# zhaodong-liu/GRAM

Hardware: AMD Instinct MI355X
Metric: users/sec @ beam=20 top-20 gen, Beauty T5-base; Recall@5 parity (higher is better)
Workload: dtype f16x3

## Files before the change

### gram_amd/csrc/gemm.hip

```cpp
#include <stdlib.h>
#include <type_traits>

#include "common.h"
#include "prof.h"

namespace {

#ifndef GRAM_PP_ABL
#define GRAM_PP_ABL 0
#endif
__device__ unsigned long long g_pp_clk[2];
constexpr int BN = 128, BK = 64;

enum { V_DMA_M64 = 31, V_DMA = 1, V_DMA_M256 = 3, V_PP = 22, V_RING_M64 = 33, V_RING_M128 = 34 };
int g_force_variant = -1;
int g_stagger = 0;
int g_pp_entry_delay = 0;
int g_pp_clk_on = 0;


__device__ __forceinline__ int swz(int row, int chunk) { return row * 128 + ((chunk ^ ((row >> 1) & 7)) << 4); }

struct EpiArgs {
  void* C;
// ... 713 lines not shown
                                       (__attribute__((address_space(3))) void*)(sw + (wave * WG + i) * 1024), 16, 0, 0);
  };

  f32x4 acc[TNW][4];
#pragma unroll
  for (int i = 0; i < TNW; ++i)
#pragma unroll
    for (int j = 0; j < 4; ++j) acc[i][j] = (f32x4){0.f, 0.f, 0.f, 0.f};

  const int nkt = K / BK;
  float rs4[4];
  if constexpr (NST >= 3) {
    constexpr int Q = AG + WG;
    static_assert(Q * (NST - 2) <= 63, "counted vmcnt");
    const char* abase = reinterpret_cast<const char*>(A + (size_t)m0 * lda);
    const char* wbase = reinterpret_cast<const char*>(W + (size_t)n0 * K);
    uint32_t a_off[AG], w_off[WG];
#pragma unroll
    for (int i = 0; i < AG; ++i) {
      const int row = (wave * AG + i) * 8 + (lane >> 3);
      a_off[i] = (uint32_t)(min(m0 + row, M - 1) - m0) * (uint32_t)lda * 2u + (uint32_t)(((lane & 7) ^ ((row >> 1) & 7)) * 16);
    }
#pragma unroll
    for (int i = 0; i < WG; ++i) {
      const int row = (wave * WG + i) * 8 + (lane >> 3);
      w_off[i] = (uint32_t)row * (uint32_t)K * 2u + (uint32_t)(((lane & 7) ^ ((row >> 1) & 7)) * 16);
    }
    const uint32_t lds0 = (uint32_t)(uintptr_t)(__attribute__((address_space(3))) char*)smem;
    const int uwave = __builtin_amdgcn_readfirstlane(wave);
    int i_slot = 0, i_kt = 0;
    auto issue = [&]() {
      const uint32_t sa = lds0 + (uint32_t)i_slot * STAGE, sw = sa + A_BYTES;
      const char* asrc = abase + (size_t)i_kt * (BK * 2);
      const char* wsrc = wbase + (size_t)i_kt * (BK * 2);
#pragma unroll
      for (int i = 0; i < AG; ++i) dma16_asm(sa + (uwave * AG + i) * 1024, a_off[i], asrc);
#pragma unroll
      for (int i = 0; i < WG; ++i) dma16_asm(sw + (uwave * WG + i) * 1024, w_off[i], wsrc);
      ++i_kt;
      i_slot = i_slot + 1 == NST ? 0 : i_slot + 1;
    };
    const int npro = min(NST - 1, nkt);
    for (int kt = 0; kt < npro; ++kt) issue();
    load_row_scales(ep, m0 + wm * 64, r16, M, rs4, n0 == 0 && wn == 0);
    int c_slot = 0;
    for (int kt = 0; kt < nkt; ++kt) {
      wait_later<Q>(min(NST - 2, nkt - 1 - kt));
      gram_sync();
      if (kt + NST - 1 < nkt) issue();
      compute_tile<TNW, X3>(smem + c_slot * STAGE, smem + c_slot * STAGE + A_BYTES, wm, wn, r16, g, acc);
      c_slot = c_slot + 1 == NST ? 0 : c_slot + 1;
    }
    gram_sync();
  } else {
  load_row_scales(ep, m0 + wm * 64, r16, M, rs4, n0 == 0 && wn == 0);
  if constexpr (NST == 1) {
    for (int kt = 0; kt < nkt; ++kt) {
      dma(kt, 0);
      gram_sync();
      compute_tile<TNW, X3>(smem, smem + A_BYTES, wm, wn, r16, g, acc);
      gram_sync();
    }
  } else {
    dma(0, 0);
    gram_sync();
    for (int kt = 0; kt < nkt; ++kt) {
      const int st = kt & 1;
      if (kt + 1 < nkt) dma(kt + 1, st ^ 1);
      compute_tile<TNW, X3>(smem + st * STAGE, smem + st * STAGE + A_BYTES, wm, wn, r16, g, acc);
      gram_sync();
    }
  }
  }
  if constexpr ((EPI == GRAM_EPI_F32_ADD || EPI == GRAM_EPI_F32) && TNW == 4 && NST != 2) {
    if (ep.nt & 4) {
      epilogue_rows64<EPI>(acc, smem + wave * 4096, m0, n0, wm, wn, lane, M, ep);
      return;
    }
  }
  epilogue<EPI, TNW>(acc, m0, n0, wm, wn, r16, g, M, ep, rs4);
}

constexpr int PP_KV_K = 100, PP_KV_V = 101;
__device__ __forceinline__ void pp_barrier() {
  asm volatile("s_barrier" ::: "memory");
  gram_chaos_point();
}

struct PPOut {
  char* c;
  char* xb;
  float* ss;
  const float* xs;
  uint32_t ldc_b;
  uint32_t ldx_b;
  uint32_t ss_nblk;
  int rows;
  int split;
  long c_ps_b;
  bool inter;
  bool nt;
  float scale;
  long q_ps;
  uint32_t q_step;
};
template <int EPI, bool FULL>
__device__ __forceinline__ void pp_store_rows_impl(f32x4 (&acc)[4][8], int j0, char* patch, const PPOut& o, int lane_, const float* rs) {
  static_assert(EPI == GRAM_EPI_BF16 || EPI == GRAM_EPI_BF16_RELU, "16-bit outputs only: the fp32 outputs go through pp_store_tile_f32");
  int lane = lane_;
  asm volatile("" : "+v"(lane));
  const int r16 = lane & 15, g = lane >> 4;
#pragma unroll
  for (int jj = 0; jj < 2; ++jj) {
    const int j = j0 + jj;
    const float sc = (rs ? rs[j * 16 + r16] : 1.f) * o.scale;
    f32x4 v[4];
#pragma unroll
    for (int i = 0; i < 4; ++i) {
      v[i] = acc[i][j] * sc;
      if constexpr (EPI == GRAM_EPI_BF16_RELU) {
#pragma unroll
        for (int e = 0; e < 4; ++e) v[i][e] = fmaxf(v[i][e], 0.f);
      }
    }
    uint2 pcs[2][4];
    if (o.split == 2) {
#pragma unroll
      for (int i = 0; i < 4; ++i) split2x4(v[i], pcs[0][i], pcs[1][i]);
    } else {
#pragma unroll
      for (int i = 0; i < 4; ++i) pcs[0][i] = pcs[1][i] = pack_bf16x4(v[i]);
    }
    for (int pc = 0; pc < o.split; ++pc) {
#pragma unroll
      for (int i = 0; i < 4; ++i) {
        const int chunk = (i * 2 + (g >> 1)) ^ (r16 & 7);
        *reinterpret_cast<uint2*>(patch + r16 * 128 + chunk * 16 + (g & 1) * 8) = pc == 0 ? pcs[0][i] : pcs[1][i];
      }
      __builtin_amdgcn_wave_barrier();
#pragma unroll
      for (int it = 0; it < 2; ++it) {
        const int row = it * 8 + (lane >> 3), c = lane & 7;
        const uint4 val = *reinterpret_cast<const uint4*>(patch + row * 128 + ((c ^ (row & 7)) * 16));
        const int mr = j * 16 + row;
        const uint32_t coff = o.inter ? (uint32_t)((c >> 2) * 128 + pc * 64 + (c & 3) * 16) : (uint32_t)(c * 16);
        if ((FULL || mr < o.rows) && (!(GRAM_PP_ABL & 16) || o.rows < -12345))
          store16(o.c + (o.inter ? 0 : pc * o.c_ps_b) + ((uint32_t)mr * o.ldc_b + coff), val, o.nt);
      }
      __builtin_amdgcn_wave_barrier();
    }
  }
}

template <int EPI>
__device__ __forceinline__ void pp_store_tile_f32(f32x4 (&acc)[4][8], char* patch, const PPOut& o, int lane_) {
  int lane = lane_;
  asm volatile("" : "+v"(lane));
  const int r16 = lane & 15, g = lane >> 4;
#pragma unroll
  for (int half = 0; half < 2; ++half) {
    f32x4 res[16];
    float xsl = 1.f;
    if constexpr (EPI == GRAM_EPI_F32_ADD) {
#pragma unroll
      for (int q = 0; q < 16; ++q) res[q] = (f32x4){0.f, 0.f, 0.f, 0.f};
      if (o.rows > 0 && o.xs) xsl = o.xs[min(half * 64 + lane, o.rows - 1)];
      if (o.rows > 0) {
#pragma unroll
        for (int q = 0; q < 16; ++q) {
          const int mr = min(half * 64 + q * 4 + (lane >> 4), o.rows - 1);
          res[q] = *reinterpret_cast<const f32x4*>(o.c + ((uint32_t)mr * o.ldc_b + (lane & 15) * 16));
        }
      }
    }
#pragma unroll
    for (int p = 0; p < 4; ++p) {
      const int j = half * 4 + p;
#pragma unroll
      for (int i = 0; i < 4; ++i) *reinterpret_cast<f32x4*>(patch + r16 * 256 + (((i * 4 + g) ^ r16) * 16)) = acc[i][j];
      __builtin_amdgcn_wave_barrier();
      float ssq4[4];
#pragma unroll
      for (int it = 0; it < 4; ++it) {
        const int row = it * 4 + (lane >> 4), c = lane & 15;
        f32x4 val = *reinterpret_cast<const f32x4*>(patch + row * 256 + ((c ^ row) * 16)) * o.scale;
        const int mr = j * 16 + row;
        float ssq = 0.f;
        const float xs_row = __shfl(xsl, p * 16 + it * 4 + (lane >> 4), 64);
        if (mr < o.rows && (!(GRAM_PP_ABL & 16) || o.rows < -12345)) {
          f32x4* pc = reinterpret_cast<f32x4*>(o.c + ((uint32_t)mr * o.ldc_b + c * 16));
          if constexpr (EPI == GRAM_EPI_F32_ADD) val += res[p * 4 + it];
          if (!(GRAM_PP_ABL & 32) || o.rows < -12345) *pc = val;
          if constexpr (EPI == GRAM_EPI_F32_ADD) {
            if (o.xb) {
              const f32x4 xv = val * xs_row;
              if (o.split == 2) {
                uint2 p0, p1;
                split2x4(xv, p0, p1);
                const bool odd = c & 1;
                const uint2 send = odd ? p0 : p1;
                uint2 recv;
                recv.x = (uint32_t)__builtin_amdgcn_mov_dpp((int)send.x, 0xB1, 0xF, 0xF, true);
                recv.y = (uint32_t)__builtin_amdgcn_mov_dpp((int)send.y, 0xB1, 0xF, 0xF, true);
                const uint4 out = odd ? make_uint4(recv.x, recv.y, p1.x, p1.y) : make_uint4(p0.x, p0.y, recv.x, recv.y);
                const uint32_t xoff = (uint32_t)((c >> 3) * 128 + (odd ? 64 : 0) + ((c & 6) * 8));
                *reinterpret_cast<uint4*>(o.xb + ((uint32_t)mr * o.ldx_b + xoff)) = out;
              } else {
                *reinterpret_cast<uint2*>(o.xb + ((uint32_t)mr * o.ldx_b + (uint32_t)(c * 8))) = pack_bf16x4(xv);
              }
              ssq = sumsq4(val);
            }
          }
        }
        ssq4[it] = ssq;
      }
      if constexpr (EPI == GRAM_EPI_F32_ADD) {
        if (o.ss) {
#pragma unroll
          for (int sh = 1; sh < 16; sh <<= 1)
#pragma unroll
            for (int it = 0; it < 4; ++it) ssq4[it] += __shfl_xor(ssq4[it], sh, 64);
          const int cc = lane & 15;
          const float mine = cc == 0 ? ssq4[0] : cc == 1 ? ssq4[1] : cc == 2 ? ssq4[2] : ssq4[3];
          const int mr = j * 16 + cc * 4 + (lane >> 4);
          if (cc < 4 && mr < o.rows) o.ss[(uint32_t)mr * o.ss_nblk] = mine;
        }
      }
      __builtin_amdgcn_wave_barrier();
    }
  }
}

template <int EPI>
__device__ __forceinline__ void pp_store_rows(f32x4 (&acc)[4][8], int j0, char* patch, const PPOut& o, int lane, const float* rs) {
  if (o.rows >= 128) pp_store_rows_impl<EPI, true>(acc, j0, patch, o, lane, rs);
  else pp_store_rows_impl<EPI, false>(acc, j0, patch, o, lane, rs);
}

template <int EPI, bool X3 = false>
__global__ __launch_bounds__(512, 1) void gemm_pp_kernel(const p16* __restrict__ A, const p16* __restrict__ W, int M, int N,
                                                         int K, int lda, EpiArgs ep, int ntiles, int stagger) {
  constexpr int TB = 256, HT = 16384;
  constexpr bool F32OUT = EPI == GRAM_EPI_F32 || EPI == GRAM_EPI_F32_ADD;
  constexpr bool KV = EPI == PP_KV_K || EPI == PP_KV_V;
  constexpr bool TRALL = EPI == PP_KV_V;
  constexpr int PATCH = 4096;
  constexpr bool LSE = EPI == GRAM_EPI_F32_LSE;
  constexpr bool TEND = F32OUT || LSE || X3;
  constexpr int RS_OFF = 8 * HT + 4 * PATCH;
  extern __shared__ __attribute__((aligned(16))) char smem[];
  const int tid = threadIdx.x;
  const int lane = tid & 63;
  const int wave = __builtin_amdgcn_readfirstlane(tid >> 6);
  const int wr = wave >> 2, wc = wave & 3;
  const int r16 = lane & 15, g = lane >> 4;
  const int ntn = KV ? N / TB / 2 : (N + TB - 1) / TB;
  auto nt_of = [&](int ntl) {
    if constexpr (KV) {
      const int it = ep.inner >> 8, blk = (int)udiv_magic((uint32_t)ntl, (uint32_t)it, ep.mg_it);
      return blk * 2 * it + (TRALL ? it : 0) + (ntl - blk * it);
    } else {
      return ntl;
    }
  };
  const int G = gridDim.x;
  const int slot = xcd_remap();
  const int xcd = blockIdx.x & 7;
  if (slot >= ntiles) return;
  const int nkt = K / BK;
  const uint32_t lds0 = (uint32_t)(uintptr_t)(__attribute__((address_space(3))) char*)smem;
  const uint32_t wave_lds = __builtin_amdgcn_readfirstlane(lds0 + wave * 2048);
  const char* const Ab = reinterpret_cast<const char*>(A);
  const char* const Wb = reinterpret_cast<const char*>(W);
  char* const patch = smem + 8 * HT + (F32OUT ? wave * PATCH : TEND ? wave * 2048 : (wave & 3) * PATCH);
  const bool has_rs = !F32OUT && ep.ss_in != nullptr;

  const int gm = (stagger >> 16) & 0xff;
  const bool clk_on = (stagger >> 30) & 1;
#ifdef GRAM_CHAOS
  const int entry_delay = (stagger >> 24) & 0x3f;
#endif
  stagger &= 0xffff;
  auto decode = [&](int tile, int& mt, int& nr) {
    if (gm <= 1) {
      mt = tile / ntn;
      nr = tile - mt * ntn;
    } else {
      const int per = gm * ntn, grp = tile / per, first = grp * gm;
      const int gs = min(gm, (M + TB - 1) / TB - first);
      const int rem = tile - grp * per;
      nr = rem / gs;
      mt = first + (rem - nr * gs);
    }
  };
  int c_tile = slot, c_kt = 0;
  const char *c_A, *c_W;
  uint32_t offA[2][2], offW[2], offW2[LSE ? 2 : 1];
  if constexpr (!LSE) {
#pragma unroll
    for (int p = 0; p < 2; ++p) {
      const int r = (wave * 2 + p) * 8 + (lane >> 3);
      const int chunk = (lane & 7) ^ ((r >> 1) & 7);
      offW[p] = ((uint32_t)((r >> 5) * 64 + (r & 31)) * (uint32_t)K + chunk * 8) * 2u;
    }
  }
  auto set_offsets = [&]() {
    int mt, nr;
    decode(c_tile, mt, nr);
    const int nt = nt_of(nr);
    c_A = Ab + (size_t)mt * TB * lda * 2;
    c_W = Wb + (size_t)nt * TB * K * 2;
    const int mleft = M - 1 - mt * TB;
    int ln = lane;
    asm volatile("" : "+v"(ln));
#pragma unroll
    for (int p = 0; p < 2; ++p) {
      const int r = (wave * 2 + p) * 8 + (ln >> 3);
      const int chunk = (ln & 7) ^ ((r >> 1) & 7);
      const int arow = (r >> 6) * 128 + (r & 63);
      offA[0][p] = ((uint32_t)min(arow, mleft) * (uint32_t)lda + chunk * 8) * 2u;
      offA[1][p] = ((uint32_t)min(arow + 64, mleft) * (uint32_t)lda + chunk * 8) * 2u;
      if constexpr (LSE) {
        const int wleft = N - 1 - nt * TB, wrow = (r >> 5) * 64 + (r & 31);
        offW[p] = ((uint32_t)min(wrow, wleft) * (uint32_t)K + chunk * 8) * 2u;
        offW2[p] = ((uint32_t)min(wrow + 32, wleft) * (uint32_t)K + chunk * 8) * 2u;
      }
    }
  };
  auto advance = [&]() {
    if (++c_kt == nkt) {
      c_kt = 0;
      if (c_tile + G < ntiles) c_tile += G;
      set_offsets();
    }
  };
  bool abl_loop = false;
  auto issue = [&](int t, int par) {
    if ((GRAM_PP_ABL & 2) && abl_loop) return;
    {
      const uint32_t dst = wave_lds + (par * 4 + t) * HT;
      if (t == 0 || t == 3) {
        const char* base = c_A + c_kt * (BK * 2);
        dma16_asm(dst, offA[t == 3][0], base);
        dma16_asm(dst + 1024, offA[t == 3][1], base);
      } else {
        if constexpr (LSE) {
          const char* base = c_W + c_kt * (BK * 2);
          dma16_asm(dst, t == 2 ? offW2[0] : offW[0], base);
          dma16_asm(dst + 1024, t == 2 ? offW2[1] : offW[1], base);
        } else {
          const char* base = c_W + c_kt * (BK * 2) + (t == 2 ? (size_t)32 * K * 2 : 0);
          dma16_asm(dst, offW[0], base);
          dma16_asm(dst + 1024, offW[1], base);
        }
      }
    }
  };

  f32x4 acc[4][8];
  p16x8 fa[2][4], fw[2][2][2];
  const char* const a_base[2] = {smem + swz(wr * 64 + r16, g), smem + swz(wr * 64 + r16, 4 + g)};
  const char* const w_base[2] = {smem + swz(wc * 32 + r16, g), smem + swz(wc * 32 + r16, 4 + g)};
  auto read_a = [&](int par, int mq) {
    if ((GRAM_PP_ABL & 4) && abl_loop) return;
    {
#pragma unroll
      for (int ks = 0; ks < 2; ++ks)
#pragma unroll
        for (int j = 0; j < 4; ++j)
          fa[ks][j] = *reinterpret_cast<const p16x8*>(a_base[ks] + (par * 4 + (mq ? 3 : 0)) * HT + j * 2048);
    }
  };
  auto read_w = [&](int par, int nq) {
    if ((GRAM_PP_ABL & 4) && abl_loop) return;
    {
#pragma unroll
      for (int ks = 0; ks < 2; ++ks)
#pragma unroll
        for (int i = 0; i < 2; ++i)
          fw[nq][ks][i] = *reinterpret_cast<const p16x8*>(w_base[ks] + (par * 4 + 1 + nq) * HT + i * 2048);
    }
  };
  constexpr int NMQ = X3 ? 24 : 16;
  auto mfma_q = [&](auto TRc, int mq, int nq, int n) {
    const int pr = n >> 3, i = (n >> 2) & 1, j = n & 3;
    const int ka = X3 ? (pr == 1 ? 1 : 0) : pr, kw = X3 ? (pr == 0 ? 1 : 0) : pr;
    f32x4& c = acc[nq * 2 + i][mq * 4 + j];
    if constexpr (decltype(TRc)::value) c = mfma16(fa[ka][j], fw[nq][kw][i], c);
    else c = mfma16(fw[nq][kw][i], fa[ka][j], c);
  };
  auto mma = [&](int mq, int nq, auto TRc) {
    __builtin_amdgcn_sched_barrier(0);
    __builtin_amdgcn_s_setprio(1);
#pragma unroll
    for (int n = 0; n < NMQ; ++n) mfma_q(TRc, mq, nq, n);
    __builtin_amdgcn_s_setprio(0);
    __builtin_amdgcn_sched_barrier(0);
    pp_barrier();
  };
  auto mma_st = [&](int mq, int nq, auto TRc, auto J0c, const PPOut& o, const float* rs, auto FULLc) {
    constexpr bool FULL = decltype(FULLc)::value;
// ... 11 lines not shown
    const char* const wbase = patch + lr * 128 + (((lg >> 1) ^ (lr & 1)) * 16) + (lg & 1) * 8;
    const char* const gbase = patch + (ln >> 3) * 128 + (((ln & 7) ^ ((ln >> 3) & 7)) * 16);
    const int mr0 = J0 * 16 + (ln >> 3);
    const uint32_t voff0 = (uint32_t)mr0 * o.ldc_b + (ln & 7) * 16;
    auto get = [&](int it) { return *reinterpret_cast<const uint4*>(gbase + it * 1024); };
    auto put = [&](int it, const uint4& v) {
      if (FULL || mr0 + it * 8 < o.rows) {
        uint4* dst = reinterpret_cast<uint4*>(o.c + (voff0 + (uint32_t)(it * 8) * o.ldc_b));
        typedef unsigned int u32x4 __attribute__((ext_vector_type(4)));
        __builtin_nontemporal_store(__builtin_bit_cast(u32x4, v), reinterpret_cast<u32x4*>(dst));
      }
    };
    __builtin_amdgcn_sched_barrier(0);
    __builtin_amdgcn_s_setprio(1);
#pragma unroll
    for (int n = 0; n < 16; ++n) {
      mfma_q(TRc, mq, nq, n);
      if (n < 8 && (n & 1)) {
#pragma unroll
        for (int pc = n - 1; pc <= n; ++pc) {
          const int jj = pc >> 2, pi = pc & 3;
          f32x4 v = acc[pi][J0 + jj] * sc[jj];
          if constexpr (EPI == GRAM_EPI_BF16_RELU) {
#pragma unroll
            for (int e = 0; e < 4; ++e) v[e] = fmaxf(v[e], 0.f);
          }
          *reinterpret_cast<uint2*>(const_cast<char*>(wbase) + jj * 2048 + ((pi * 32) ^ wx)) = pack_bf16x4(v);
        }
      }
      if (n == 7) __builtin_amdgcn_wave_barrier();
      if (n == 8) pva = get(0);
      if (n == 10) {
        put(0, pva);
        pva = get(1);
      }
      if (n == 12) {
        put(1, pva);
        pva = get(2);
      }
      if (n == 14) {
        put(2, pva);
        pva = get(3);
      }
      __builtin_amdgcn_sched_barrier(0);
    }
    __builtin_amdgcn_s_setprio(0);
    put(3, pva);
    asm volatile("s_waitcnt lgkmcnt(0)" ::: "memory");
    __builtin_amdgcn_sched_barrier(0);
    pp_barrier();
  };
  struct KVLoc {
    char* kb;
    char* vb;
    int mblk;
  };
  auto kv_locate = [&](int tm0, int tn0, int J0) {
    KVLoc q;
    q.mblk = tm0 + wr * 128 + J0 * 16;
    int b_, s0;
    if (ep.pmap) {
      const int pp = (int)udiv_magic((uint32_t)q.mblk >> 5, (uint32_t)ep.pL >> 5, ep.mg_pL32), l = q.mblk - pp * ep.pL, flat = ep.pmap[pp];
      b_ = (int)udiv_magic((uint32_t)flat, (uint32_t)ep.pN, ep.mg_pN);
      s0 = (flat - b_ * ep.pN) * ep.pL + l;
    } else {
      b_ = (int)udiv_magic((uint32_t)q.mblk >> 5, (uint32_t)ep.S >> 5, ep.mg_S32);
      s0 = q.mblk - b_ * ep.S;
    }
    const int n = tn0 + wc * 64, lw = (int)udiv_magic((uint32_t)n >> 8, (uint32_t)ep.inner >> 8, ep.mg_it);
    const size_t head = ((size_t)(lw >> 1) * ep.B + b_) * ep.H + ((n - lw * ep.inner) >> 6);
    q.kb = reinterpret_cast<char*>(ep.bank_k + (head * ep.S + s0) * 64);
    q.vb = reinterpret_cast<char*>(ep.bank_vt + (head * (size_t)(ep.S >> 5) + (size_t)(s0 >> 5)) * 2048);
    return q;
  };
  auto kv_direct = [&](auto TRc, const KVLoc& q, int jj, int pi, const f32x4& v, int lr, int lg) {
    typedef unsigned int u32x2 __attribute__((ext_vector_type(2)));
    const u32x2 pk = __builtin_bit_cast(u32x2, pack_bf16x4(v * ep.out_scale));
    if constexpr (decltype(TRc)::value) {
      const uint32_t off = ((uint32_t)(pi * 16 + lr) * 32u + jj * 16 + 4 * lg) * 2u;
      if (q.mblk + jj * 16 + 4 * lg < M) __builtin_nontemporal_store(pk, reinterpret_cast<u32x2*>(q.vb + off));
    } else {
      const uint32_t off = ((uint32_t)(jj * 16 + lr) * 64u + pi * 16 + 4 * lg) * 2u;
      if (q.mblk + jj * 16 + lr < M) __builtin_nontemporal_store(pk, reinterpret_cast<u32x2*>(q.kb + off));
    }
  };
  auto mma_vt = [&](int mq, int nq, auto TRc, auto J0c, const KVLoc& q) {
    constexpr int J0 = decltype(J0c)::value;
    int ln = lane;
    asm volatile("" : "+v"(ln));
    const int lr = ln & 15, lg = ln >> 4;
    const char* const wbase = patch + lr * 64 + (lg & 1) * 8;
    const int wsw = (lr >> 2) & 3;
    const int rd = ln >> 2, rc = ln & 3;
    const char* const gbase = patch + rd * 64 + ((rc ^ ((rd >> 2) & 3)) * 16);
    const uint32_t voff0 = ((uint32_t)rd * 32u + rc * 8) * 2u;
    uint4 pv;
    auto get = [&](int it) { return *reinterpret_cast<const uint4*>(gbase + it * 1024); };
    auto put = [&](int it, const uint4& v) {
      typedef unsigned int u32x4 __attribute__((ext_vector_type(4)));
      __builtin_nontemporal_store(__builtin_bit_cast(u32x4, v),
                                  reinterpret_cast<u32x4*>(q.vb + (voff0 + (uint32_t)(it * 1024))));
    };
    __builtin_amdgcn_sched_barrier(0);
    __builtin_amdgcn_s_setprio(1);
#pragma unroll
    for (int n = 0; n < 16; ++n) {
      mfma_q(TRc, mq, nq, n);
      if (n < 8 && (n & 1)) {
#pragma unroll
        for (int pc = n - 1; pc <= n; ++pc) {
          const int jj = pc >> 2, pi = pc & 3;
          const int chunk = (jj * 2 + (lg >> 1)) ^ wsw;
          *reinterpret_cast<uint2*>(const_cast<char*>(wbase) + pi * 1024 + chunk * 16) = pack_bf16x4(acc[pi][J0 + jj] * ep.out_scale);
        }
      }
      if (n == 7) __builtin_amdgcn_wave_barrier();
      if (n == 8) pv = get(0);
      if (n == 10) {
        put(0, pv);
        pv = get(1);
      }
      if (n == 12) {
        put(1, pv);
        pv = get(2);
      }
      if (n == 14) {
        put(2, pv);
        pv = get(3);
      }
      __builtin_amdgcn_sched_barrier(0);
    }
    __builtin_amdgcn_s_setprio(0);
    put(3, pv);
    asm volatile("s_waitcnt lgkmcnt(0)" ::: "memory");
    __builtin_amdgcn_sched_barrier(0);
    pp_barrier();
  };
  auto kv_out_k = [&](const KVLoc& q, int tm0, int J0) {
    PPOut o{};
    o.c = q.kb - (size_t)J0 * 16 * 128;
    o.ldc_b = 128;
    o.rows = M - (tm0 + wr * 128);
    o.split = 1;
    o.inter = false;
    o.nt = true;
    o.scale = ep.out_scale;
    return o;
  };
  auto end_load_slot = [&](int extra = 0) {
    if (extra == 0) asm volatile("s_waitcnt vmcnt(12)" ::: "memory");
    else if (extra == 4) asm volatile("s_waitcnt vmcnt(16)" ::: "memory");
    else if (extra == 8) asm volatile("s_waitcnt vmcnt(20)" ::: "memory");
    else if (extra == 12) asm volatile("s_waitcnt vmcnt(24)" ::: "memory");
    else asm volatile("s_waitcnt vmcnt(28)" ::: "memory");
    asm volatile("s_waitcnt lgkmcnt(0)" ::: "memory");
    __builtin_amdgcn_sched_barrier(0);
    pp_barrier();
  };
  auto zero_half = [&](int mq) {
#pragma unroll
    for (int i = 0; i < 4; ++i)
#pragma unroll
      for (int j = 0; j < 4; ++j) acc[i][mq * 4 + j] = (f32x4){0.f, 0.f, 0.f, 0.f};
  };

  if (stagger > 0) {
    const int ph = (stagger & 0x8000) ? xcd : (slot & 7);
    stagger &= 0x7fff;
    const int units = (ph * stagger * nkt) >> 3;
    for (int i = 0; i < units; ++i) __builtin_amdgcn_s_sleep(8);
  }
  set_offsets();
  issue(1, 0);
  issue(0, 0);
  issue(2, 0);
  issue(3, 0);
  advance();
  issue(2, 1);
  issue(0, 1);
  issue(1, 1);
  issue(3, 1);
  advance();
  asm volatile("s_waitcnt vmcnt(12)" ::: "memory");
  pp_barrier();
#ifdef GRAM_CHAOS
  if (wr == 1) for (int i = 0; i < entry_delay; ++i) __builtin_amdgcn_s_sleep(8);
#endif
  read_w(0, 0);
  asm volatile("s_waitcnt lgkmcnt(0)" ::: "memory");
  pp_barrier();
  if (wr == 1) pp_barrier();

  int tile = slot;
  int m0, n0, tpar = 0;
  constexpr int ESZ = F32OUT ? 4 : 2;
  int pm0 = 0, pn0 = 0;
  auto make_out = [&](int tm0, int tn0) {
    PPOut o;
    const size_t mf = (size_t)tm0 + wr * 128;
    const int nf = tn0 + wc * 64;
    o.inter = !F32OUT && ep.c_inter != 0;
    o.c = reinterpret_cast<char*>(ep.C) + (mf * ep.ldc + (o.inter ? 2 * nf : nf)) * ESZ;
    o.xb = ep.xb_out ? reinterpret_cast<char*>(ep.xb_out) + (mf * ep.ldc + nf) * 2 * ep.split : nullptr;
    o.ss = ep.ss_out ? ep.ss_out + mf * ep.ss_out_nblk + (nf >> 6) : nullptr;
    o.xs = ep.xs_in && ep.xb_out ? ep.xs_in + mf : nullptr;
    o.ldc_b = ep.ldc * ESZ;
    o.ldx_b = ep.ldc * 2 * ep.split;
    o.ss_nblk = ep.ss_out_nblk;
    o.rows = M - (int)mf;
    o.split = ep.split;
    o.c_ps_b = ep.c_pstride * 2;
    o.nt = (ep.nt & 8) != 0;
    o.scale = ep.out_scale;
    o.q_ps = o.inter ? 64 : o.c_ps_b;
    o.q_step = o.inter ? 128u : 64u;
    return o;
  };
  auto run_slot = [&](int mq, int nq, bool job, auto J0c, int tm0, int tn0, const float* rs) {
    constexpr int J0 = decltype(J0c)::value;
    if constexpr (KV) {
      using TR = std::integral_constant<bool, TRALL>;
      job = job && tm0 + wr * 128 + J0 * 16 < M;
      if (!job) {
        mma(mq, nq, TR{});
      } else {
        const KVLoc q = kv_locate(tm0, tn0, J0);
        if constexpr (TRALL) mma_vt(mq, nq, TR{}, J0c, q);
        else mma_st(mq, nq, TR{}, J0c, kv_out_k(q, tm0, J0), nullptr, std::false_type{});
      }
    } else {
      if (job) {
        const PPOut o = make_out(tm0, tn0);
        if (o.rows >= 128) mma_st(mq, nq, std::false_type{}, J0c, o, rs, std::true_type{});
        else mma_st(mq, nq, std::false_type{}, J0c, o, rs, std::false_type{});
      }
      else mma(mq, nq, std::false_type{});
    }
  };
  bool pending = false;
  zero_half(0);
  zero_half(1);
  abl_loop = true;
  const unsigned long long clk_t0 = __builtin_amdgcn_s_memtime(), clk_r0 = __builtin_amdgcn_s_memrealtime();
  while (true) {
    {
      int mt, nr;
      decode(tile, mt, nr);
      const int nt = nt_of(nr);
      m0 = mt * TB;
      n0 = nt * TB;
    }
    const float* rs_cur = has_rs ? reinterpret_cast<const float*>(smem + RS_OFF) + tpar * 256 + wr * 128 : nullptr;
    const float* rs_prev = has_rs ? reinterpret_cast<const float*>(smem + RS_OFF) + (tpar ^ 1) * 256 + wr * 128 : nullptr;
    for (int kt = 0; kt < nkt; kt += 2) {
      const bool first = kt == 0, last = kt + 2 >= nkt;
      const bool pf = !TEND && !F32OUT && !KV && first && pending && M - (pm0 + wr * 128) >= 128;
      const bool lf = !TEND && !F32OUT && !KV && last && M - (m0 + wr * 128) >= 128;
      const bool st_prev = first && pending, st_cur = last;
      read_a(0, 0);
      issue(1, 0);
      end_load_slot(pf ? 8 : 0);
      run_slot(0, 0, !TEND && st_prev, std::integral_constant<int, 4>{}, pm0, pn0, rs_prev);
      read_w(0, 1);
      issue(0, 0);
      end_load_slot(pf ? 12 : 0);
      run_slot(0, 1, !TEND && st_prev, std::integral_constant<int, 6>{}, pm0, pn0, rs_prev);
      read_a(0, 1);
      if (first) {
        if constexpr (!TEND) zero_half(1);
        if (has_rs && wave < 4) {
          int ln = lane;
          asm volatile("" : "+v"(ln));
          dma4_asm(lds0 + RS_OFF + tpar * 1024 + wave * 256, (uint32_t)min(m0 + wave * 64 + ln, M - 1) * 4u,
                   reinterpret_cast<const char*>(ep.ss_in));
        }
      }
      issue(2, 0);
      end_load_slot(pf ? 16 : 0);
      run_slot(1, 1, false, std::integral_constant<int, 0>{}, 0, 0, nullptr);
      read_w(1, 1);
      issue(3, 0);
      end_load_slot(pf ? 16 : 0);
      run_slot(1, 0, false, std::integral_constant<int, 0>{}, 0, 0, nullptr);
      advance();
      read_a(1, 0);
      issue(2, 1);
      end_load_slot(pf ? 16 : 0);
      run_slot(0, 1, false, std::integral_constant<int, 0>{}, 0, 0, nullptr);
      read_w(1, 0);
      issue(0, 1);
      end_load_slot(pf ? 12 : 0);
      run_slot(0, 0, false, std::integral_constant<int, 0>{}, 0, 0, nullptr);
      read_a(1, 1);
      issue(1, 1);
      end_load_slot(pf ? 8 : 0);
      run_slot(1, 0, !TEND && st_cur, std::integral_constant<int, 0>{}, m0, n0, rs_cur);
      read_w(0, 0);
      issue(3, 1);
      end_load_slot((pf ? 4 : 0) + (lf ? 4 : 0));
      run_slot(1, 1, !TEND && st_cur, std::integral_constant<int, 2>{}, m0, n0, rs_cur);
      if (last && !TEND) zero_half(0);
      advance();
    }
    const bool more = tile + G < ntiles;
    if constexpr (TEND) {
      if (wr == 0) pp_barrier();
      if constexpr ((GRAM_PP_ABL & 1) != 0) {
        float t = 0.f;
#pragma unroll
        for (int i = 0; i < 4; ++i)
#pragma unroll
          for (int j = 0; j < 8; ++j) t += (acc[i][j][0] + acc[i][j][1]) + (acc[i][j][2] + acc[i][j][3]);
        if (t == 12345.678f) reinterpret_cast<float*>(ep.C ? ep.C : ep.lse_part ? (void*)ep.lse_part : (void*)ep.bank_k)[lane] = t;
      } else if constexpr (LSE) {
        const int blk = (n0 + wc * 64) >> 6;
        if (blk < ep.lse_nblk) {
#pragma unroll
          for (int j = 0; j < 8; ++j) {
#pragma unroll
            for (int i = 0; i < 4; ++i) acc[i][j] *= ep.out_scale;
            float mx = -INFINITY;
#pragma unroll
            for (int i = 0; i < 4; ++i)
#pragma unroll
              for (int e = 0; e < 4; ++e) mx = fmaxf(mx, acc[i][j][e]);
            mx = fmaxf(mx, __shfl_xor(mx, 16, 64));
            mx = fmaxf(mx, __shfl_xor(mx, 32, 64));
            float sm = 0.f;
#pragma unroll
            for (int i = 0; i < 4; ++i)
#pragma unroll
              for (int e = 0; e < 4; ++e) sm += __expf(acc[i][j][e] - mx);
            sm += __shfl_xor(sm, 16, 64);
            sm += __shfl_xor(sm, 32, 64);
            const int m = m0 + wr * 128 + j * 16 + r16;
            if (g == 0 && m < M) *reinterpret_cast<float2*>(ep.lse_part + ((size_t)m * ep.lse_nblk + blk) * 2) = make_float2(mx, sm);
          }
        }
      } else if constexpr (KV) {
        char* const kvpatch = smem + 8 * HT + wave * 4096;
#pragma unroll
        for (int J0 = 0; J0 < 8; J0 += 2) {
          if (m0 + wr * 128 + J0 * 16 < M) {
            const KVLoc q = kv_locate(m0, n0, J0);
            if constexpr (!TRALL) {
              PPOut o = kv_out_k(q, m0, J0);
              o.split = ep.split;
              o.c_ps_b = ep.bank_pstride * 2;
              pp_store_rows_impl<GRAM_EPI_BF16, false>(acc, J0, kvpatch, o, lane, nullptr);
            } else {
              int ln = lane;
              asm volatile("" : "+v"(ln));
              const int lr = ln & 15, lg = ln >> 4;
              const int wsw = (lr >> 2) & 3, rd = ln >> 2, rc = ln & 3;
              char* const wbase = kvpatch + lr * 64 + (lg & 1) * 8;
              const char* const gbase = kvpatch + rd * 64 + ((rc ^ ((rd >> 2) & 3)) * 16);
              const uint32_t voff0 = ((uint32_t)rd * 32u + rc * 8) * 2u;
              char* vb = q.vb;
#pragma unroll
              for (int pcs = 0; pcs < 8; ++pcs) acc[pcs & 3][J0 + (pcs >> 2)] *= ep.out_scale;
              for (int pc = 0; pc < ep.split; ++pc) {
#pragma unroll
                for (int pcs = 0; pcs < 8; ++pcs) {
                  const int jj = pcs >> 2, pi = pcs & 3;
                  f32x4& v = acc[pi][J0 + jj];
                  uint2 pk;
                  if (pc == 0) {
                    uint2 lo;
                    split2x4(v, pk, lo);
                    v[0] = __uint_as_float(lo.x);
                    v[1] = __uint_as_float(lo.y);
                  } else {
                    pk = make_uint2(__float_as_uint(v[0]), __float_as_uint(v[1]));
                  }
                  *reinterpret_cast<uint2*>(wbase + pi * 1024 + (((jj * 2 + (lg >> 1)) ^ wsw) * 16)) = pk;
                }
                __builtin_amdgcn_wave_barrier();
#pragma unroll
                for (int it = 0; it < 4; ++it) {
                  typedef unsigned int u32x4 __attribute__((ext_vector_type(4)));
                  const uint4 val = *reinterpret_cast<const uint4*>(gbase + it * 1024);
                  __builtin_nontemporal_store(__builtin_bit_cast(u32x4, val),
                                              reinterpret_cast<u32x4*>(vb + (voff0 + (uint32_t)(it * 1024))));
                }
                __builtin_amdgcn_wave_barrier();
                vb += ep.bank_pstride * 2;
              }
            }
          }
        }
      } else {
        const PPOut o = make_out(m0, n0);
        if constexpr (F32OUT) {
          pp_store_tile_f32<EPI>(acc, patch, o, lane);
        } else {
          pp_store_rows<EPI>(acc, 0, patch, o, lane, rs_cur);
          pp_store_rows<EPI>(acc, 2, patch, o, lane, rs_cur);
          pp_store_rows<EPI>(acc, 4, patch, o, lane, rs_cur);
          pp_store_rows<EPI>(acc, 6, patch, o, lane, rs_cur);
        }
      }
      zero_half(0);
      zero_half(1);
      pp_barrier();
      if (more && wr == 1) pp_barrier();
    }
    pending = true;
    pm0 = m0;
    pn0 = n0;
    tpar ^= 1;
    if (!more) break;
    tile += G;
  }
  if (clk_on && tid == 0) {
    atomicAdd(&g_pp_clk[0], (unsigned long long)__builtin_amdgcn_s_memtime() - clk_t0);
    atomicAdd(&g_pp_clk[1], (unsigned long long)__builtin_amdgcn_s_memrealtime() - clk_r0);
  }
  if constexpr (!TEND) {
    if (wr == 0) pp_barrier();
  }
  asm volatile("s_waitcnt vmcnt(0)" ::: "memory");
  pp_barrier();
  if constexpr (!TEND) {
    const float* rs_prev = has_rs ? reinterpret_cast<const float*>(smem + RS_OFF) + (tpar ^ 1) * 256 + wr * 128 : nullptr;
    if constexpr (KV) {
#pragma unroll
      for (int J0 = 4; J0 < 8; J0 += 2) {
        if (pm0 + wr * 128 + J0 * 16 < M) {
          const KVLoc q = kv_locate(pm0, pn0, J0);
#pragma unroll
          for (int pc = 0; pc < 8; ++pc)
            kv_direct(std::integral_constant<bool, TRALL>{}, q, pc >> 2, pc & 3, acc[pc & 3][J0 + (pc >> 2)], r16, g);
        }
      }
    } else {
      const PPOut o = make_out(pm0, pn0);
      pp_store_rows<EPI>(acc, 4, smem + wave * 4096, o, lane, rs_prev);
      pp_store_rows<EPI>(acc, 6, smem + wave * 4096, o, lane, rs_prev);
    }
  }
}

template <int EPI, bool X3 = false>
int launch_pp(const void* A, const void* W, int M, int N, int K, int lda, EpiArgs ep, hipStream_t st) {
  if constexpr (EPI == GRAM_EPI_KV_BANK) {
    const int r = launch_pp<PP_KV_K, X3>(A, W, M, N, K, lda, ep, st);
    return r ? r : launch_pp<PP_KV_V, X3>(A, W, M, N, K, lda, ep, st);
  } else {
  if ((ep.split > 1) != X3) return GRAM_E_ARG;
  constexpr int smem = 8 * 16384 + 8 * 4096;
  if ((EPI == GRAM_EPI_F32_LSE ? N % 128 : N % 256) || (K / BK) % 2 || K / BK < 4 || (ep.ss_in && ep.ss_nblk != 0)) return GRAM_E_ARG;
  if (EPI == GRAM_EPI_F32_LSE && ep.C) return GRAM_E_ARG;
  if ((size_t)256 * lda * 2 >= (1ull << 31) || (size_t)256 * K * 2 >= (1ull << 31) || (size_t)256 * ep.ldc * 4 >= (1ull << 31))
    return GRAM_E_ARG;
  {
    if constexpr (EPI == PP_KV_K || EPI == PP_KV_V) {
      if (ep.inner % 256 || ((ep.pmap ? ep.pL : ep.S) % 32) || M % 32) return GRAM_E_ARG;
      if (ep.S > 4096 || (ep.pmap && (ep.pL > 4096 || ep.pN > 64 || (long)ep.B * ep.pN >= (1l << 26))) || M >= (1 << 30)) return GRAM_E_ARG;
      ep.mg_pL32 = magic_u32(ep.pmap ? ep.pL >> 5 : 1);
      ep.mg_S32 = magic_u32(ep.S >> 5);
      ep.mg_pN = magic_u32(ep.pmap ? ep.pN : 1);
      ep.mg_it = magic_u32(ep.inner >> 8);
    }
    const int ntiles = ((EPI == PP_KV_K || EPI == PP_KV_V) ? N / 512 : (N + 255) / 256) * ((M + 255) / 256);
    static int n_cu = 0;
    if (n_cu == 0) {
      int dev = 0;
      hipDeviceProp_t prop;
      if (hipGetDevice(&dev) != hipSuccess || hipGetDeviceProperties(&prop, dev) != hipSuccess) return GRAM_E_ARG;
      n_cu = prop.multiProcessorCount;
    }
    const int nblocks = ntiles < n_cu ? ntiles : n_cu;
    static bool attr_set = false;
    if (!attr_set) {
      hipError_t e = hipFuncSetAttribute(reinterpret_cast<const void*>(gemm_pp_kernel<EPI, X3>),
                                         hipFuncAttributeMaxDynamicSharedMemorySize, smem);
      if (e != hipSuccess) return (int)e;
      attr_set = true;
    }
    static const int gm_set = getenv("GRAM_GEMM_GROUPM") ? atoi(getenv("GRAM_GEMM_GROUPM")) : -1;
    const int gm_env = gm_set >= 0 ? gm_set : (ep.split > 1 ? 4 : 6);
    const int ntn_ = ntiles / ((M + 255) / 256);
    const int gm = ntn_ >= 8 && gm_env > 1 && gm_env < 256 ? gm_env : 0;
    static const int nt7 = getenv("GRAM_GEMM_NT7") ? atoi(getenv("GRAM_GEMM_NT7")) : 0;
    if (nt7) ep.nt |= 8;
    static const int stagger_env = getenv("GRAM_GEMM_STAGGER") ? atoi(getenv("GRAM_GEMM_STAGGER")) : -1;
    static const int stagger_xcd = getenv("GRAM_GEMM_STAGGER_XCD") ? atoi(getenv("GRAM_GEMM_STAGGER_XCD")) : 0;
    const int stagger = (stagger_env >= 0 ? stagger_env : g_stagger) | (stagger_xcd ? 0x8000 : 0);
    hipLaunchKernelGGL((gemm_pp_kernel<EPI, X3>), dim3(nblocks), dim3(512), smem, st, (const p16*)A, (const p16*)W, M, N, K, lda,
                       ep, ntiles, (stagger & 0xffff) | (gm << 16) | ((g_pp_entry_delay & 0x3f) << 24) | (g_pp_clk_on ? 1 << 30 : 0));
    GRAM_CHECK_LAUNCH();
    return 0;
  }
  }
}

int pp_min_m() {
  static const int v = getenv("GRAM_GEMM_PP_MINM") ? atoi(getenv("GRAM_GEMM_PP_MINM")) : 32768;
  return v;
}
int pick_variant(int M, int N, int K) {
  if (g_force_variant >= 0) return g_force_variant;
  const long tiles256 = (long)((M + 255) / 256) * (N / BN);
  static const long pp_min_tiles = getenv("GRAM_GEMM_PP_MINTILES") ? atol(getenv("GRAM_GEMM_PP_MINTILES")) : 1536;
  if (N % 256 == 0 && M >= pp_min_m() && (tiles256 >= pp_min_tiles * (long)pp_min_m() / 32768 || K >= 2048)) return V_PP;
  if (tiles256 >= 2048) return V_DMA_M256;
  static const int use_ring = getenv("GRAM_GEMM_RING") ? atoi(getenv("GRAM_GEMM_RING")) : 1;
  if (use_ring) {
    if ((long)((M + 63) / 64) * (N / BN) <= 256) return V_RING_M64;
    if ((long)((M + 127) / 128) * (N / BN) <= 256) return V_RING_M128;
  }
  static const int m64_max = getenv("GRAM_GEMM_M64_MAXTILES") ? atoi(getenv("GRAM_GEMM_M64_MAXTILES")) : 256;
  if ((long)((M + 127) / 128) * (N / BN) < m64_max) return V_DMA_M64;
  return V_DMA;
}

template <int EPI, int WM, int NST, bool X3, int TNW = 4>
int launch_dma(const void* A, const void* W, int M, int N, int K, int lda, EpiArgs ep, hipStream_t st) {
  constexpr int TBM = 64 * WM, TBN = 32 * TNW;
  constexpr int smem = NST * (TBM + TBN) * BK * 2;
  if (N % TBN) return GRAM_E_ARG;
  const int nblocks = (N / TBN) * ((M + TBM - 1) / TBM);
  static bool attr_set = false;
  if (!attr_set && smem > 48 * 1024) {
    hipError_t e = hipFuncSetAttribute(reinterpret_cast<const void*>(gemm_dma_kernel<EPI, WM, NST, TNW, X3>),
                                       hipFuncAttributeMaxDynamicSharedMemorySize, smem);
    if (e != hipSuccess) return (int)e;
    attr_set = true;
  }
  static const int rows_env = getenv("GRAM_GEMM_DMAROWS") ? atoi(getenv("GRAM_GEMM_DMAROWS")) : 1;
  if (rows_env) ep.nt |= 4;
  hipLaunchKernelGGL((gemm_dma_kernel<EPI, WM, NST, TNW, X3>), dim3(nblocks), dim3(WM * 128), smem, st, (const p16*)A, (const p16*)W,
                     M, N, K, lda, ep);
  GRAM_CHECK_LAUNCH();
  return 0;
}

constexpr int V_SKINNY = 30, V_STREAM = 32;

template <int EPI, bool X3>
int launch_dma_variant(int v, const void* A, const void* W, int M, int N, int K, int lda, const EpiArgs& ep, hipStream_t st) {
  switch (v) {
    case V_DMA_M64: return launch_dma<EPI, 1, 1, X3>(A, W, M, N, K, lda, ep, st);
    case V_RING_M64: return launch_dma<EPI, 1, 6, X3>(A, W, M, N, K, lda, ep, st);
    case V_RING_M128: return launch_dma<EPI, 2, 4, X3>(A, W, M, N, K, lda, ep, st);
    case V_PP:
    case V_DMA_M256: return launch_dma<EPI, 4, 1, X3>(A, W, M, N, K, lda, ep, st);
// ... 203 lines not shown
```

Baseline: 3164.

## Pipeline x3 16-bit epilogue stores across the tile and defer their vmcnt waits

Adds a tile-wide epilogue for the split-precision (x3) 16-bit output path. Each 16-row group's LDS patch read is double-buffered, so global stores of one group overlap the packing of the next, and the K and generic bf16 outputs are written in one pass instead of four per-row-pair calls. The next tile's first load waits are relaxed to vmcnt(44) so those outstanding stores do not block the mainloop. This adds register pressure and relies on the hand-counted vmcnt value being correct.

```diff
diff --git a/gram_amd/csrc/gemm.hip b/gram_amd/csrc/gemm.hip
--- a/gram_amd/csrc/gemm.hip
+++ b/gram_amd/csrc/gemm.hip
@@ -889,6 +889,63 @@
   }
 }
 
+template <int EPI, int NJ, bool FULL, int NT>
+__device__ __forceinline__ void pp_store_tile_x3(f32x4 (&acc)[4][8], int j0, char* patch, const PPOut& o, char* const (&cb)[NJ / 2],
+                                                 int lane_, const float* rs) {
+  static_assert(EPI == GRAM_EPI_BF16 || EPI == GRAM_EPI_BF16_RELU, "16-bit outputs only");
+  int lane = lane_;
+  asm volatile("" : "+v"(lane));
+  const int r16 = lane & 15, g = lane >> 4;
+  float sc[NJ];
+#pragma unroll
+  for (int jj = 0; jj < NJ; ++jj) sc[jj] = (rs ? rs[(j0 + jj) * 16 + r16] : 1.f) * o.scale;
+  char* wr_[4];
+#pragma unroll
+  for (int i = 0; i < 4; ++i) wr_[i] = patch + r16 * 128 + (((i * 2 + (g >> 1)) ^ (r16 & 7)) * 16) + (g & 1) * 8;
+  const int row0 = lane >> 3, c = lane & 7;
+  const char* const rd = patch + row0 * 128 + ((c ^ (row0 & 7)) * 16);
+  const uint32_t voff = (uint32_t)row0 * o.ldc_b + (o.inter ? (uint32_t)((c >> 2) * 128 + (c & 3) * 16) : (uint32_t)(c * 16));
+  const long pstep = o.inter ? 64 : o.c_ps_b;
+  uint2 pcs[2][4];
+  uint4 buf[2][2];
+  constexpr int NG = NJ * 2;
+#pragma unroll
+  for (int s = 0; s <= NG; ++s) {
+    if (s < NG) {
+      const int jj = s >> 1, pc = s & 1;
+      if (pc == 0) {
+#pragma unroll
+        for (int i = 0; i < 4; ++i) {
+          f32x4 v = acc[i][j0 + jj] * sc[jj];
+          if constexpr (EPI == GRAM_EPI_BF16_RELU) {
+#pragma unroll
+            for (int e = 0; e < 4; ++e) v[e] = fmaxf(v[e], 0.f);
+          }
+          split2x4(v, pcs[0][i], pcs[1][i]);
+        }
+      }
+#pragma unroll
+      for (int i = 0; i < 4; ++i) *reinterpret_cast<uint2*>(wr_[i]) = pcs[pc][i];
+      __builtin_amdgcn_wave_barrier();
+#pragma unroll
+      for (int it = 0; it < 2; ++it) buf[s & 1][it] = *reinterpret_cast<const uint4*>(rd + it * 1024);
+      __builtin_amdgcn_wave_barrier();
+      __builtin_amdgcn_sched_barrier(0);
+    }
+    if (s > 0) {
+      const int t = s - 1, jj = t >> 1, pc = t & 1;
+      char* const base = cb[jj >> 1] + pc * pstep;
+#pragma unroll
+      for (int it = 0; it < 2; ++it) {
+        const int mr = (jj & 1) * 16 + it * 8;
+        if ((FULL || (j0 + jj) * 16 + it * 8 + row0 < o.rows) && (!(GRAM_PP_ABL & 16) || o.rows < -12345))
+          store16(base + ((uint32_t)mr * o.ldc_b + voff), buf[t & 1][it], NT < 0 ? o.nt : NT != 0);
+      }
+      __builtin_amdgcn_sched_barrier(0);
+    }
+  }
+}
+
 template <int EPI>
 __device__ __forceinline__ void pp_store_tile_f32(f32x4 (&acc)[4][8], char* patch, const PPOut& o, int lane_) {
   int lane = lane_;
@@ -984,6 +1041,7 @@
   constexpr int PATCH = 4096;
   constexpr bool LSE = EPI == GRAM_EPI_F32_LSE;
   constexpr bool TEND = F32OUT || LSE || X3;
+  constexpr bool T16 = X3 && !F32OUT && !LSE;
   constexpr int RS_OFF = 8 * HT + 4 * PATCH;
   extern __shared__ __attribute__((aligned(16))) char smem[];
   const int tid = threadIdx.x;
@@ -1301,6 +1359,7 @@
     else if (extra == 4) asm volatile("s_waitcnt vmcnt(16)" ::: "memory");
     else if (extra == 8) asm volatile("s_waitcnt vmcnt(20)" ::: "memory");
     else if (extra == 12) asm volatile("s_waitcnt vmcnt(24)" ::: "memory");
+    else if (extra == 32) asm volatile("s_waitcnt vmcnt(44)" ::: "memory");
     else asm volatile("s_waitcnt vmcnt(28)" ::: "memory");
     asm volatile("s_waitcnt lgkmcnt(0)" ::: "memory");
     __builtin_amdgcn_sched_barrier(0);
@@ -1387,6 +1446,7 @@
     }
   };
   bool pending = false;
+  int st_extra = 0;
   zero_half(0);
   zero_half(1);
   abl_loop = true;
@@ -1406,13 +1466,14 @@
       const bool pf = !TEND && !F32OUT && !KV && first && pending && M - (pm0 + wr * 128) >= 128;
       const bool lf = !TEND && !F32OUT && !KV && last && M - (m0 + wr * 128) >= 128;
       const bool st_prev = first && pending, st_cur = last;
+      const int ex = (T16 && first) ? st_extra : 0;
       read_a(0, 0);
       issue(1, 0);
-      end_load_slot(pf ? 8 : 0);
+      end_load_slot(pf ? 8 : ex);
       run_slot(0, 0, !TEND && st_prev, std::integral_constant<int, 4>{}, pm0, pn0, rs_prev);
       read_w(0, 1);
       issue(0, 0);
-      end_load_slot(pf ? 12 : 0);
+      end_load_slot(pf ? 12 : ex);
       run_slot(0, 1, !TEND && st_prev, std::integral_constant<int, 6>{}, pm0, pn0, rs_prev);
       read_a(0, 1);
       if (first) {
@@ -1425,16 +1486,16 @@
         }
       }
       issue(2, 0);
-      end_load_slot(pf ? 16 : 0);
+      end_load_slot(pf ? 16 : ex);
       run_slot(1, 1, false, std::integral_constant<int, 0>{}, 0, 0, nullptr);
       read_w(1, 1);
       issue(3, 0);
-      end_load_slot(pf ? 16 : 0);
+      end_load_slot(pf ? 16 : ex);
       run_slot(1, 0, false, std::integral_constant<int, 0>{}, 0, 0, nullptr);
       advance();
       read_a(1, 0);
       issue(2, 1);
-      end_load_slot(pf ? 16 : 0);
+      end_load_slot(pf ? 16 : ex);
       run_slot(0, 1, false, std::integral_constant<int, 0>{}, 0, 0, nullptr);
       read_w(1, 0);
       issue(0, 1);
@@ -1488,6 +1549,21 @@
         }
       } else if constexpr (KV) {
         char* const kvpatch = smem + 8 * HT + wave * 4096;
+        const bool kfull = M - (m0 + wr * 128) >= 128;
+        st_extra = kfull && !(GRAM_PP_ABL & 17) ? 32 : 0;
+        bool stored = false;
+        if constexpr (!TRALL) {
+          if (kfull) {
+            char* cb[4];
+#pragma unroll
+            for (int P = 0; P < 4; ++P) cb[P] = kv_locate(m0, n0, 2 * P).kb;
+            PPOut o = kv_out_k(KVLoc{}, m0, 0);
+            o.c_ps_b = ep.bank_pstride * 2;
+            pp_store_tile_x3<GRAM_EPI_BF16, 8, true, 1>(acc, 0, kvpatch, o, cb, lane, nullptr);
+            stored = true;
+          }
+        }
+        if (!stored)
 #pragma unroll
         for (int J0 = 0; J0 < 8; J0 += 2) {
           if (m0 + wr * 128 + J0 * 16 < M) {
@@ -1496,7 +1572,8 @@
               PPOut o = kv_out_k(q, m0, J0);
               o.split = ep.split;
               o.c_ps_b = ep.bank_pstride * 2;
-              pp_store_rows_impl<GRAM_EPI_BF16, false>(acc, J0, kvpatch, o, lane, nullptr);
+              char* const cb[1] = {q.kb};
+              pp_store_tile_x3<GRAM_EPI_BF16, 2, false, 1>(acc, J0, kvpatch, o, cb, lane, nullptr);
             } else {
               int ln = lane;
               asm volatile("" : "+v"(ln));
@@ -1542,6 +1619,14 @@
         const PPOut o = make_out(m0, n0);
         if constexpr (F32OUT) {
           pp_store_tile_f32<EPI>(acc, patch, o, lane);
+        } else if constexpr (X3) {
+          char* cb[4];
+#pragma unroll
+          for (int P = 0; P < 4; ++P) cb[P] = o.c + (size_t)P * 32 * o.ldc_b;
+          st_extra = o.rows >= 128 && !(GRAM_PP_ABL & 17) ? 32 : 0;
+          if (o.rows < 128) pp_store_tile_x3<EPI, 8, false, -1>(acc, 0, patch, o, cb, lane, rs_cur);
+          else if (o.nt) pp_store_tile_x3<EPI, 8, true, 1>(acc, 0, patch, o, cb, lane, rs_cur);
+          else pp_store_tile_x3<EPI, 8, true, 0>(acc, 0, patch, o, cb, lane, rs_cur);
         } else {
           pp_store_rows<EPI>(acc, 0, patch, o, lane, rs_cur);
           pp_store_rows<EPI>(acc, 2, patch, o, lane, rs_cur);
```

Result: no change. 3174 (median of 6 runs) (+0.3%).
